# disanda/Deep-GAN-Encoders

Measured on AMD Instinct MI355X. Metric: encoder-train images/sec (E_align_s2 step, StyleGAN2 FFHQ-1024), higher is better.
Workload: dtype bf16; 1 GPU; E_align_s2 two-phase step, StyleGAN2-1024 G (train mode) + BE(startf=16, L=9) + LPIPS-VGG16 (seeded stand-in weights), batch 8/GPU; global_batch=8, img_size=1024, parallelism=dp1

## Files before the change

deep-gan-encoders_amd/csrc/enc_bwd_kernels.hip:

```cpp
#include <stdlib.h>
#include "common.h"
#include "../../include/dge_hip.h"

template <int NTAP>
__device__ __forceinline__ void wgrad_flush(const f32x16_t (&acc)[NTAP], float* smem, float* __restrict__ dW, int o0, int i0,
                                            int Co, int Ci, int tid, int lane, int wave) {
    float* red = smem;
    float* stage = smem + 4096;
#pragma unroll
    for (int t = 0; t < NTAP; t++) {
        __syncthreads();
#pragma unroll
        for (int r = 0; r < 16; r++) red[wave * 1024 + r * 64 + lane] = acc[t][r];
        __syncthreads();
#pragma unroll
        for (int q = 0; q < 4; q++) {
            const int e = tid + q * 256;
            const int r = e >> 6, ln = e & 63;
            const int ol = (r & 3) + 8 * (r >> 2) + 4 * (ln >> 5), il = ln & 31;
            stage[(ol * 32 + il) * NTAP + t] = (red[e] + red[1024 + e]) + (red[2048 + e] + red[3072 + e]);
        }
    }
    __syncthreads();
    const int ni = (Ci - i0 < 32 ? Ci - i0 : 32) * NTAP;
    if (det_on()) {
        const int L = 1024 * NTAP, nslots = gridDim.y;
        float* slot = det_slot(blockIdx.x, gridDim.x, blockIdx.y, nslots, L);
        for (int idx = tid; idx < L; idx += 256) slot[idx] = stage[idx];
        if (det_arrive_wg(blockIdx.x, nslots)) {
            for (int idx = tid; idx < L; idx += 256) {
                const int ol = idx / (32 * NTAP), j = idx - ol * (32 * NTAP);
                if (o0 + ol < Co && j < ni) dW[((size_t)(o0 + ol) * Ci + i0) * NTAP + j] += det_sum(blockIdx.x, nslots, L, idx);
            }
        }
        return;
    }
    for (int idx = tid; idx < 1024 * NTAP; idx += 256) {
        const int ol = idx / (32 * NTAP), j = idx - ol * (32 * NTAP);
        if (o0 + ol < Co && j < ni) atomicAdd(dW + ((size_t)(o0 + ol) * Ci + i0) * NTAP + j, stage[idx]);
    }
}

template <typename T, int KS>
__global__ __launch_bounds__(256) void conv_wgrad_kernel(const T* __restrict__ g, const T* __restrict__ X,
                                                          const float* __restrict__ sc, const float* __restrict__ sh,
                                                          float* __restrict__ dW, int B, int H, int W, int Co, int Ci,
                                                          int tiles_x, int tiles_y, int ntile_groups) {
    constexpr int TH = 8, TW = 16, HALO = KS / 2, HH = TH + 2 * HALO, HW = TW + 2 * HALO;
    constexpr int EP = Elem<T>::PER16;
    constexpr int ES = (int)sizeof(T);
    constexpr int NTAP = KS * KS;
    constexpr int GPIT = TH * TW + 16 / ES;
    constexpr int XROW = 24 * 2 / ES >= 24 ? 24 : 24;
    constexpr int XPIT = HH * XROW + 16 / ES;
    constexpr int LG_BYTES = 32 * GPIT * ES, LX_BYTES = 32 * XPIT * ES;
    constexpr int FL_BYTES = (4096 + 1024 * NTAP) * 4;
    constexpr int SM_BYTES = (LG_BYTES + LX_BYTES) > FL_BYTES ? (LG_BYTES + LX_BYTES) : FL_BYTES;
    __shared__ __attribute__((aligned(16))) unsigned char smem[SM_BYTES];
    T* lg = (T*)smem;
    T* lx = (T*)(smem + LG_BYTES);
    const int tid = threadIdx.x, lane = tid & 63, wave = tid >> 6;
    const int n_it = (Ci + 31) / 32;
    const int o0 = (blockIdx.x / n_it) * 32, i0 = (blockIdx.x % n_it) * 32;
    f32x16_t acc[NTAP];
#pragma unroll
    for (int t = 0; t < NTAP; t++)
#pragma unroll
        for (int r = 0; r < 16; r++) acc[t][r] = 0.f;
    const int ntiles = tiles_x * tiles_y * B;
    constexpr int CPR = 32 / EP;
    constexpr int NG = (TH * TW * CPR + 255) / 256, NX = (HH * HW * CPR + 255) / 256;
    __shared__ float laff[64];
    const int m = lane & 31, kg = lane >> 5;
    uint4 greg[NG], xreg[NX];
    auto load_tile = [&](int tile) {
        const int tx_i = tile % tiles_x, ty_i = (tile / tiles_x) % tiles_y, b = tile / (tiles_x * tiles_y);
        const int x0 = tx_i * TW, y0 = ty_i * TH;
#pragma unroll
        for (int k = 0; k < NG; k++) {
            const int idx = tid + k * 256;
            const int pix = idx % (TH * TW), c = idx / (TH * TW), gy = y0 + pix / TW, gx = x0 + pix % TW;
            uint4 v = make_uint4(0, 0, 0, 0);
            if (idx < TH * TW * CPR && gy < H && gx < W && o0 + c * EP < Co)
                v = *(const uint4*)(g + ((size_t)(b * H + gy) * W + gx) * Co + o0 + c * EP);
            greg[k] = v;
        }
#pragma unroll
        for (int k = 0; k < NX; k++) {
            const int idx = tid + k * 256;
            const int pix = idx % (HH * HW), c = idx / (HH * HW), hy = pix / HW, hx = pix % HW;
            const int gy = y0 + hy - HALO, gx = x0 + hx - HALO;
            uint4 v = make_uint4(0, 0, 0, 0);
            if (idx < HH * HW * CPR && gy >= 0 && gy < H && gx >= 0 && gx < W && i0 + c * EP < Ci)
                v = *(const uint4*)(X + ((size_t)(b * H + gy) * W + gx) * Ci + i0 + c * EP);
            xreg[k] = v;
        }
    };
    int b_aff = -1;
    if ((int)blockIdx.y < ntiles) load_tile(blockIdx.y);
    for (int tile = blockIdx.y; tile < ntiles; tile += ntile_groups) {
        const int tx_i = tile % tiles_x, ty_i = (tile / tiles_x) % tiles_y, b = tile / (tiles_x * tiles_y);
        const int x0 = tx_i * TW, y0 = ty_i * TH;
        __syncthreads();
        if (sc && b != b_aff) {
            if (tid < 64) {
                const int ch = i0 + (tid & 31);
                laff[tid] = ch < Ci ? (tid < 32 ? sc[b * Ci + ch] : sh[b * Ci + ch]) : 0.f;
            }
            b_aff = b;
            __syncthreads();
        }
#pragma unroll
        for (int k = 0; k < NG; k++) {
            const int idx = tid + k * 256;
            if (idx < TH * TW * CPR) {
                const int pix = idx % (TH * TW), c = idx / (TH * TW);
                const T* e = (const T*)&greg[k];
#pragma unroll
                for (int q = 0; q < EP; q++) lg[(c * EP + q) * GPIT + pix] = e[q];
            }
        }
#pragma unroll
        for (int k = 0; k < NX; k++) {
            const int idx = tid + k * 256;
            if (idx < HH * HW * CPR) {
                const int pix = idx % (HH * HW), c = idx / (HH * HW), hy = pix / HW, hx = pix % HW;
                const int gy = y0 + hy - HALO, gx = x0 + hx - HALO;
                uint4 v = xreg[k];
                if (sc && gy >= 0 && gy < H && gx >= 0 && gx < W) {
                    float f[EP];
                    unpack16(v, f, (T*)nullptr);
#pragma unroll
                    for (int q = 0; q < EP; q++) f[q] = f[q] * laff[c * EP + q] + laff[32 + c * EP + q];
                    v = pack16(f, (T*)nullptr);
                }
                const T* e = (const T*)&v;
#pragma unroll
                for (int q = 0; q < EP; q++) lx[(c * EP + q) * XPIT + hy * XROW + hx] = e[q];
            }
        }
        __syncthreads();
        if (tile + ntile_groups < ntiles) load_tile(tile + ntile_groups);
        constexpr int RW = TH / 4;
#pragma unroll
        for (int rr = 0; rr < RW; rr++) {
            const int row = RW * wave + rr;
            if constexpr (sizeof(T) == 2) {
                const uint4 a = *(const uint4*)(lg + m * GPIT + row * TW + kg * 8);
#pragma unroll
                for (int dy = 0; dy < KS; dy++) {
                    const T* xr = lx + m * XPIT + (row + dy) * XROW + kg * 8;
                    const uint4 v0 = *(const uint4*)xr;
                    if constexpr (KS == 3) {
                        const uint32_t v1 = *(const uint32_t*)(xr + 8);
                        const uint4 b1 = make_uint4(__builtin_amdgcn_alignbit(v0.y, v0.x, 16), __builtin_amdgcn_alignbit(v0.z, v0.y, 16),
                                                    __builtin_amdgcn_alignbit(v0.w, v0.z, 16), __builtin_amdgcn_alignbit(v1, v0.w, 16));
                        const uint4 b2 = make_uint4(v0.y, v0.z, v0.w, v1);
                        acc[dy * 3 + 0] = __builtin_amdgcn_mfma_f32_32x32x16_bf16(*(const bf16x8_t*)&a, *(const bf16x8_t*)&v0, acc[dy * 3 + 0], 0, 0, 0);
                        acc[dy * 3 + 1] = __builtin_amdgcn_mfma_f32_32x32x16_bf16(*(const bf16x8_t*)&a, *(const bf16x8_t*)&b1, acc[dy * 3 + 1], 0, 0, 0);
                        acc[dy * 3 + 2] = __builtin_amdgcn_mfma_f32_32x32x16_bf16(*(const bf16x8_t*)&a, *(const bf16x8_t*)&b2, acc[dy * 3 + 2], 0, 0, 0);
                    } else {
                        acc[0] = __builtin_amdgcn_mfma_f32_32x32x16_bf16(*(const bf16x8_t*)&a, *(const bf16x8_t*)&v0, acc[0], 0, 0, 0);
                    }
                }
            } else {
                const float* ar = (const float*)lg + m * GPIT + row * TW + kg * 8;
                float af[8];
                *(uint4*)&af[0] = *(const uint4*)ar; *(uint4*)&af[4] = *(const uint4*)(ar + 4);
#pragma unroll
                for (int dy = 0; dy < KS; dy++) {
                    const float* xr = (const float*)lx + m * XPIT + (row + dy) * XROW + kg * 8;
                    float xf[12];
                    *(uint4*)&xf[0] = *(const uint4*)xr; *(uint4*)&xf[4] = *(const uint4*)(xr + 4);
                    if constexpr (KS == 3) *(uint4*)&xf[8] = *(const uint4*)(xr + 8);
#pragma unroll
                    for (int dx = 0; dx < KS; dx++)
#pragma unroll
                        for (int j = 0; j < 8; j++)
                            acc[dy * KS + dx] = __builtin_amdgcn_mfma_f32_32x32x2f32(af[j], xf[j + dx], acc[dy * KS + dx], 0, 0, 0);
                }
            }
        }
    }
    wgrad_flush<NTAP>(acc, (float*)smem, dW, o0, i0, Co, Ci, tid, lane, wave);
}

typedef short v4s_t __attribute__((ext_vector_type(4)));
template <int KS, int TH>
__global__ __launch_bounds__(256) void conv_wgrad_tr_kernel(const bf16_t* __restrict__ g, const bf16_t* __restrict__ X,
                                                             const float* __restrict__ sc, const float* __restrict__ sh,
                                                             float* __restrict__ dW, int B, int H, int W, int Co, int Ci,
                                                             int tiles_x, int tiles_y, int ntile_groups) {
    constexpr int TW = 16, HALO = KS / 2, HH = TH + 2 * HALO, HW = TW + 2 * HALO;
    constexpr int NTAP = KS * KS;
    constexpr int LG_BYTES = TH * TW * 64, LX_BYTES = (HH * HW + 4) * 64;
    constexpr int FL_BYTES = (4096 + 1024 * NTAP) * 4;
    constexpr int SM_BYTES = (LG_BYTES + LX_BYTES) > FL_BYTES ? (LG_BYTES + LX_BYTES) : FL_BYTES;
    __shared__ __attribute__((aligned(256))) unsigned char smem[SM_BYTES];
    __shared__ float laff[64];
    unsigned char* lg = smem;
    unsigned char* lx = smem + LG_BYTES;
    const int tid = threadIdx.x, lane = tid & 63;
    const int wave = __builtin_amdgcn_readfirstlane(tid >> 6);
    const int n_it = (Ci + 31) / 32;
    const int o0 = (blockIdx.x / n_it) * 32, i0 = (blockIdx.x % n_it) * 32;
    f32x16_t acc[NTAP];
#pragma unroll
    for (int t = 0; t < NTAP; t++)
#pragma unroll
        for (int r = 0; r < 16; r++) acc[t][r] = 0.f;
    const int ntiles = tiles_x * tiles_y * B;
    constexpr int NG = TH * TW * 4 / 256, NX = (HH * HW * 4 + 255) / 256;
    const int cch = tid & 3;
    const bool gc_ok = o0 + cch * 8 < Co, xc_ok = i0 + cch * 8 < Ci;
    uint4 greg[NG], xreg[NX];
    unsigned xin = 0;
    auto load_tile = [&](int tile) {
        const int tx_i = tile % tiles_x, ty_i = (tile / tiles_x) % tiles_y, b = tile / (tiles_x * tiles_y);
        const int x0 = tx_i * TW, y0 = ty_i * TH;
        const bf16_t* gb = g + (size_t)b * H * W * Co + o0 + cch * 8;
        const bf16_t* xb = X + (size_t)b * H * W * Ci + i0 + cch * 8;
#pragma unroll
        for (int k = 0; k < NG; k++) {
            const int pix = (tid >> 2) + k * 64, gy = y0 + pix / TW, gx = x0 + pix % TW;
            uint4 v = make_uint4(0, 0, 0, 0);
            if ((gy < H) & (gx < W) & gc_ok) v = *(const uint4*)(gb + (gy * W + gx) * Co);
            greg[k] = v;
        }
        xin = 0;
#pragma unroll
        for (int k = 0; k < NX; k++) {
            const int pix = (tid >> 2) + k * 64, hy = pix / HW, hx = pix % HW;
            const int gy = y0 + hy - HALO, gx = x0 + hx - HALO;
            const bool in = (pix < HH * HW) & ((unsigned)gy < (unsigned)H) & ((unsigned)gx < (unsigned)W) & xc_ok;
            uint4 v = make_uint4(0, 0, 0, 0);
            if (in) v = *(const uint4*)(xb + (gy * W + gx) * Ci);
            xin |= (in ? 1u : 0u) << k;
            xreg[k] = v;
        }
    };
    const int grp = lane >> 4, li = lane & 15;
    const int frag_off = ((grp >> 1) * 8 + (li >> 2)) * 64 + (grp & 1) * 32 + (li & 3) * 8;
    typedef __attribute__((address_space(3))) v4s_t* lds_v4s_ptr;
    auto trd = [&](const unsigned char* base, int byte_off) {
        return __builtin_amdgcn_ds_read_tr16_b64_v4i16((lds_v4s_ptr)(base + byte_off));
    };
    int b_aff = -1;
    if ((int)blockIdx.y < ntiles) load_tile(blockIdx.y);
    for (int tile = blockIdx.y; tile < ntiles; tile += ntile_groups) {
        const int b = tile / (tiles_x * tiles_y);
        __syncthreads();
        if (sc && b != b_aff) {
            if (tid < 64) {
                const int ch = i0 + (tid & 31);
                laff[tid] = ch < Ci ? (tid < 32 ? sc[b * Ci + ch] : sh[b * Ci + ch]) : 0.f;
            }
            b_aff = b;
            __syncthreads();
        }
#pragma unroll
        for (int k = 0; k < NG; k++) *(uint4*)(lg + (tid + k * 256) * 16) = greg[k];
#pragma unroll
        for (int k = 0; k < NX; k++) {
            if (NX * 256 == HH * HW * 4 || tid + k * 256 < HH * HW * 4) {
                uint4 v = xreg[k];
                if (sc && ((xin >> k) & 1u)) {
                    float f[8];
                    unpack16(v, f, (bf16_t*)nullptr);
#pragma unroll
                    for (int q = 0; q < 8; q++) f[q] = f[q] * laff[cch * 8 + q] + laff[32 + cch * 8 + q];
                    v = pack16(f, (bf16_t*)nullptr);
                }
                *(uint4*)(lx + (tid + k * 256) * 16) = v;
            }
        }
        __syncthreads();
        if (tile + ntile_groups < ntiles) load_tile(tile + ntile_groups);
        constexpr int RW = TH / 4;
#pragma unroll
        for (int rr = 0; rr < RW; rr++) {
            const int row = RW * wave + rr;
            const unsigned char* ga = lg + row * TW * 64 + frag_off;
            const v4s_t a0 = trd(ga, 0), a1 = trd(ga, 4 * 64);
            const uint2 a01 = *(const uint2*)&a0, a23 = *(const uint2*)&a1;
            const uint4 av = make_uint4(a01.x, a01.y, a23.x, a23.y);
            const bf16x8_t a = *(const bf16x8_t*)&av;
#pragma unroll
            for (int dy = 0; dy < KS; dy++) {
                const unsigned char* xa = lx + (row + dy) * HW * 64 + frag_off;
                const v4s_t q0 = trd(xa, 0), q1 = trd(xa, 4 * 64);
                const uint2 w01 = *(const uint2*)&q0, w23 = *(const uint2*)&q1;
                const uint4 v0 = make_uint4(w01.x, w01.y, w23.x, w23.y);
                if constexpr (KS == 3) {
                    const v4s_t q2 = trd(xa, 8 * 64);
                    const uint32_t w4 = (*(const uint2*)&q2).x;
                    const uint4 b1 = make_uint4(__builtin_amdgcn_alignbit(v0.y, v0.x, 16), __builtin_amdgcn_alignbit(v0.z, v0.y, 16),
                                                __builtin_amdgcn_alignbit(v0.w, v0.z, 16), __builtin_amdgcn_alignbit(w4, v0.w, 16));
                    const uint4 b2 = make_uint4(v0.y, v0.z, v0.w, w4);
                    acc[dy * 3 + 0] = __builtin_amdgcn_mfma_f32_32x32x16_bf16(a, *(const bf16x8_t*)&v0, acc[dy * 3 + 0], 0, 0, 0);
                    acc[dy * 3 + 1] = __builtin_amdgcn_mfma_f32_32x32x16_bf16(a, *(const bf16x8_t*)&b1, acc[dy * 3 + 1], 0, 0, 0);
                    acc[dy * 3 + 2] = __builtin_amdgcn_mfma_f32_32x32x16_bf16(a, *(const bf16x8_t*)&b2, acc[dy * 3 + 2], 0, 0, 0);
                } else {
                    acc[0] = __builtin_amdgcn_mfma_f32_32x32x16_bf16(a, *(const bf16x8_t*)&v0, acc[0], 0, 0, 0);
                }
            }
        }
    }
    wgrad_flush<NTAP>(acc, (float*)smem, dW, o0, i0, Co, Ci, tid, lane, wave);
}

template <typename T, int NS>
__global__ __launch_bounds__(256) void act_bwd_kernel(const T* __restrict__ gup, const T* __restrict__ a,
                                                       const float* __restrict__ noise, T* __restrict__ gpre,
                                                       float* __restrict__ red_out, int H, int W, int C, int pool, float scale, float slope) {
    constexpr int EP = Elem<T>::PER16;
    __shared__ float red[256 * NS * EP];
    const int b = blockIdx.y;
    const int cpt = C / EP, ppi = 256 / cpt;
    const int chunk = threadIdx.x % cpt, slot = threadIdx.x / cpt;
    const int HW = H * W, UW = pool ? W / 2 : W, UHW = pool ? HW / 4 : HW;
    const float raw_w = pool ? 0.25f : 1.f;
    float s[NS][EP];
#pragma unroll
    for (int k = 0; k < NS; k++)
#pragma unroll
        for (int e = 0; e < EP; e++) s[k][e] = 0.f;
    for (int p0 = blockIdx.x * ppi; p0 < HW; p0 += gridDim.x * ppi) {
        const int p = p0 + slot;
        if (slot < ppi && p < HW) {
            const int q = pool ? (p / W / 2) * UW + (p % W) / 2 : p;
            float g[EP], av[EP];
            unpack16(*(const uint4*)(gup + ((size_t)b * UHW + q) * C + chunk * EP), g, (T*)nullptr);
            unpack16(*(const uint4*)(a + ((size_t)b * HW + p) * C + chunk * EP), av, (T*)nullptr);
            const float nz = noise ? noise[(size_t)b * HW + p] : 0.f;
#pragma unroll
            for (int e = 0; e < EP; e++) {
                if constexpr (NS == 3) s[2][e] += raw_w * g[e];
                g[e] = scale * g[e] * (av[e] > 0.f ? 1.f : slope);
                s[0][e] += g[e]; s[1][e] += g[e] * nz;
            }
            *(uint4*)(gpre + ((size_t)b * HW + p) * C + chunk * EP) = pack16(g, (T*)nullptr);
        }
    }
    if (red_out) block_chan_flush<EP, NS>(s, cpt, ppi, red_out + (size_t)b * C * NS, C, red);
}

template <typename T, int NS>
__global__ __launch_bounds__(256) void act_bwd_mask_kernel(const T* __restrict__ gup, const unsigned* __restrict__ mask,
                                                            const float* __restrict__ noise, T* __restrict__ gpre,
                                                            float* __restrict__ red_out, int H, int W, int C, float scale, float slope) {
    constexpr int EP = Elem<T>::PER16;
    __shared__ float red[256 * NS * EP];
    const int b = blockIdx.y;
    const int cpt = C / EP, ppi = 256 / cpt;
    const int chunk = threadIdx.x % cpt, slot = threadIdx.x / cpt;
    const int UW = W / 2, UHW = (H / 2) * UW, HW = H * W;
    float s[NS][EP];
#pragma unroll
    for (int k = 0; k < NS; k++)
#pragma unroll
        for (int e = 0; e < EP; e++) s[k][e] = 0.f;
    const int stride = gridDim.x * ppi;
    for (int q0 = blockIdx.x * ppi; q0 < UHW; q0 += 2 * stride) {
        const int qq[2] = {q0 + slot, q0 + slot + stride};
        bool ok[2]; uint4 gv[2]; unsigned mv[2]; int p00[2]; float nzv[2][4];
#pragma unroll
        for (int h = 0; h < 2; h++) {
            ok[h] = slot < ppi && qq[h] < UHW;
            gv[h] = make_uint4(0, 0, 0, 0); mv[h] = 0; p00[h] = 0;
#pragma unroll
            for (int c4 = 0; c4 < 4; c4++) nzv[h][c4] = 0.f;
            if (ok[h]) {
                gv[h] = *(const uint4*)(gup + ((size_t)b * UHW + qq[h]) * C + chunk * EP);
                mv[h] = mask[((size_t)b * UHW + qq[h]) * cpt + chunk];
                const int oy = qq[h] / UW, ox = qq[h] - oy * UW;
                p00[h] = (2 * oy) * W + 2 * ox;
                if (noise) {
#pragma unroll
                    for (int c4 = 0; c4 < 4; c4++) nzv[h][c4] = noise[(size_t)b * HW + p00[h] + (c4 >> 1) * W + (c4 & 1)];
                }
            }
        }
#pragma unroll
        for (int h = 0; h < 2; h++) {
            if (!ok[h]) continue;
            float g[EP];
            unpack16(gv[h], g, (T*)nullptr);
            const unsigned m = mv[h];
#pragma unroll
            for (int e = 0; e < EP; e++) { if constexpr (NS == 3) s[2][e] += g[e]; g[e] *= scale; }
#pragma unroll
            for (int c4 = 0; c4 < 4; c4++) {
                const int p = p00[h] + (c4 >> 1) * W + (c4 & 1);
                const float nz = nzv[h][c4];
                float o[EP];
#pragma unroll
                for (int e = 0; e < EP; e++) {
                    o[e] = g[e] * (((m >> (c4 * EP + e)) & 1u) ? 1.f : slope);
                    s[0][e] += o[e]; s[1][e] += o[e] * nz;
                }
                *(uint4*)(gpre + ((size_t)b * HW + p) * C + chunk * EP) = pack16(o, (T*)nullptr);
            }
        }
    }
    if (red_out) block_chan_flush<EP, NS>(s, cpt, ppi, red_out + (size_t)b * C * NS, C, red);
}

__global__ void in_bwd_coef_kernel(const float* __restrict__ dots, const float* __restrict__ gms, const float* __restrict__ musig,
                                   const float* __restrict__ sc, const float* __restrict__ sh, float* __restrict__ coef,
                                   int B, int C, float inv_n, int nslot) {
    const int idx = blockIdx.x * blockDim.x + threadIdx.x;
    if (idx >= B * C) return;
    const int b = idx / C, c = idx % C;
    const float r = sc[idx], s = sh[idx];
    float S2 = 0.f, S1 = 0.f;
    if (dots) {
        const float2 ss = sum_slot_pairs(dots + (size_t)idx * 2, (size_t)B * C * 2, nslot);
        S2 = ss.x; S1 = ss.y;
    }
    const float m1 = S1 * inv_n, m2 = (r * S2 + s * S1) * inv_n;
    const float mu = musig[(size_t)b * 2 * C + c], sg = musig[(size_t)b * 2 * C + C + c];
    const float gmu = gms ? gms[(size_t)b * 2 * C + c] : 0.f, gsg = gms ? gms[(size_t)b * 2 * C + C + c] : 0.f;
    const float k = sg > 0.f ? gsg * inv_n / sg : 0.f;
    coef[(size_t)idx * 3 + 0] = r;
    coef[(size_t)idx * 3 + 1] = -r * r * m2 + k;
    coef[(size_t)idx * 3 + 2] = -r * m1 - r * m2 * s + gmu * inv_n - k * mu;
}

struct InCoefSrc { const float* dots; const float* gms; const float* musig; const float* sc; const float* sh; int nslot, B; float inv_n; };
template <typename T, bool FR>
__global__ __launch_bounds__(256) void in_bwd_kernel(const T* __restrict__ gy, const T* __restrict__ X, const float* __restrict__ coef,
                                                      const T* __restrict__ extra, const float* __restrict__ noise,
                                                      T* __restrict__ gout, float* __restrict__ red_out, int H, int W, int C,
                                                      int extra_pool, float extra_scale, int act, InCoefSrc cs,
                                                      const float* __restrict__ img, float* __restrict__ fr_out) {
    constexpr int EP = Elem<T>::PER16;
    __shared__ float red[256 * (FR ? 4 : 2) * EP];
    __shared__ float lcoef[3 * 512];
    const int b = blockIdx.y;
    const int cpt = C / EP, ppi = 256 / cpt;
    const int chunk = threadIdx.x % cpt, slot = threadIdx.x / cpt;
    const int HW = H * W, UW = extra_pool ? W / 2 : W, UHW = extra_pool ? HW / 4 : HW;
    float s[FR ? 4 : 2][EP], A[EP], Bc[EP], Cc[EP];
    if (!coef) {
        for (int c = threadIdx.x; c < C; c += 256) {
            const int idx = b * C + c;
            const float r = cs.sc[idx], sft = cs.sh[idx];
            float S2 = 0.f, S1 = 0.f;
            if (cs.dots) { const float2 ss = sum_slot_pairs(cs.dots + (size_t)idx * 2, (size_t)cs.B * C * 2, cs.nslot); S2 = ss.x; S1 = ss.y; }
            const float m1 = S1 * cs.inv_n, m2 = (r * S2 + sft * S1) * cs.inv_n;
            const float mu = cs.musig[(size_t)b * 2 * C + c], sg = cs.musig[(size_t)b * 2 * C + C + c];
            const float gmu = cs.gms ? cs.gms[(size_t)b * 2 * C + c] : 0.f, gsg = cs.gms ? cs.gms[(size_t)b * 2 * C + C + c] : 0.f;
            const float k = sg > 0.f ? gsg * cs.inv_n / sg : 0.f;
            lcoef[c * 3 + 0] = r;
            lcoef[c * 3 + 1] = -r * r * m2 + k;
            lcoef[c * 3 + 2] = -r * m1 - r * m2 * sft + gmu * cs.inv_n - k * mu;
        }
        __syncthreads();
    }
#pragma unroll
    for (int e = 0; e < EP; e++) {
// ... 231 lines not shown
            unpack16(ev[h], ex, (T*)nullptr);
            a[h][0] = a[h][1] = a[h][2] = 0.f;
            if (ok[h]) {
#pragma unroll
                for (int e = 0; e < EP; e++) {
                    float ge;
                    if constexpr (AFF) ge = A[e] * g[e];
                    else ge = A[e] * g[e] + Bc[e] * xv[e] + Cc[e];
                    if (extra) ge += extra_scale * ex[e];
                    const float gp = ge * (xv[e] > 0.f ? 1.f : 0.2f);
                    a[h][0] += gp * wr[0][e]; a[h][1] += gp * wr[1][e]; a[h][2] += gp * wr[2][e];
                    if constexpr (FR) { s[0][e] += gp * im[h][0]; s[1][e] += gp * im[h][1]; s[2][e] += gp * im[h][2]; s[3][e] += gp; }
                }
            }
        }
        for (int m = 1; m < cpt && m < 64; m <<= 1) {
#pragma unroll
            for (int h = 0; h < 2; h++)
#pragma unroll
                for (int k = 0; k < 3; k++) a[h][k] += __shfl_xor(a[h][k], m, 64);
        }
        if (cpt > 64) {
            const int wave = threadIdx.x >> 6, wpp = cpt >> 6;
            if ((threadIdx.x & 63) == 0) {
#pragma unroll
                for (int h = 0; h < 2; h++)
#pragma unroll
                    for (int k = 0; k < 3; k++) xw[(h * 4 + wave) * 3 + k] = a[h][k];
            }
            __syncthreads();
            if (chunk == 0) {
#pragma unroll
                for (int h = 0; h < 2; h++)
#pragma unroll
                    for (int k = 0; k < 3; k++) {
                        float t = 0.f;
                        for (int j = 0; j < wpp; j++) t += xw[(h * 4 + wave + j) * 3 + k];
                        a[h][k] = t;
                    }
            }
            __syncthreads();
        }
        if (chunk == 0) {
#pragma unroll
            for (int h = 0; h < 2; h++) {
                if (!ok[h]) continue;
#pragma unroll
                for (int k = 0; k < 3; k++) gimg[((size_t)b * 3 + k) * HW + pp[h]] = a[h][k];
            }
        }
    }
    if constexpr (FR) block_chan_flush<EP, 4>(s, cpt, ppi, fr_out + (size_t)b * C * 4, C, red);
}

template <typename T>
__global__ __launch_bounds__(256) void nearest_up2_kernel(const T* __restrict__ x, T* __restrict__ y, int H, int W, int C, float scale, long total16) {
    constexpr int EP = Elem<T>::PER16;
    const int cpt = C / EP;
    for (long idx = blockIdx.x * 256L + threadIdx.x; idx < total16; idx += (long)gridDim.x * 256) {
        const int chunk = idx % cpt;
        const long pix = idx / cpt;
        const int ox = pix % (2 * W), oy = (pix / (2 * W)) % (2 * H);
        const long b = pix / ((long)4 * H * W);
        float v[EP];
        unpack16(*(const uint4*)(x + ((b * H + (oy >> 1)) * W + (ox >> 1)) * C + chunk * EP), v, (T*)nullptr);
#pragma unroll
        for (int e = 0; e < EP; e++) v[e] *= scale;
        *(uint4*)(y + pix * C + chunk * EP) = pack16(v, (T*)nullptr);
    }
}

__global__ void dense_wgrad_kernel(const float* __restrict__ gy, int ldgy, const float* __restrict__ x, int ldx,
                                   float* __restrict__ gW, float* __restrict__ gb, int B, int O, int I, int accumulate) {
    const long idx = blockIdx.x * 256L + threadIdx.x;
    if (idx >= (long)O * I) return;
    const int o = idx / I, i = idx % I;
    float s = 0.f, sb = 0.f;
    for (int b = 0; b < B; b++) { const float g = gy[(size_t)b * ldgy + o]; s += g * x[(size_t)b * ldx + i]; sb += g; }
    gW[idx] = accumulate ? gW[idx] + s : s;
    if (gb && i == 0) gb[o] = accumulate ? gb[o] + sb : sb;
}

struct HeadEntry { const float* W; long moff, woff; int I, gcol, boff, pad; const float* bias; };
__global__ __launch_bounds__(1024) void head_bwd_data_kernel(const HeadEntry* __restrict__ tab, const float* __restrict__ g, int ldg,
                                                             float* __restrict__ gms_all, int O) {
    __shared__ float part[16][64];
    const HeadEntry e = tab[blockIdx.z];
    const int lane = threadIdx.x & 63, wave = threadIdx.x >> 6;
    const int k = blockIdx.x * 64 + lane, b = blockIdx.y;
    if (blockIdx.x * 64 >= e.I) return;
    const int per = (O + 15) / 16, o0 = wave * per, o1 = min(O, o0 + per);
    float acc[8];
#pragma unroll
    for (int j = 0; j < 8; j++) acc[j] = 0.f;
    if (k < e.I) {
        const float* gr = g + (size_t)b * ldg + e.gcol;
        int o = o0;
        for (; o + 7 < o1; o += 8) {
#pragma unroll
            for (int j = 0; j < 8; j++) acc[j] += gr[o + j] * e.W[(size_t)(o + j) * e.I + k];
        }
        for (; o < o1; o++) acc[0] += gr[o] * e.W[(size_t)o * e.I + k];
    }
    part[wave][lane] = ((acc[0] + acc[1]) + (acc[2] + acc[3])) + ((acc[4] + acc[5]) + (acc[6] + acc[7]));
    __syncthreads();
    if (wave == 0 && k < e.I) {
        float s = 0.f;
#pragma unroll
        for (int j = 0; j < 16; j++) s += part[j][lane];
        gms_all[e.moff + (size_t)b * e.I + k] = s;
    }
}
__global__ void head_bwd_param_kernel(const HeadEntry* __restrict__ tab, const float* __restrict__ g, int ldg,
                                      const float* __restrict__ musig_all, float* __restrict__ gw_all, float* __restrict__ gb_all,
                                      int B, int O) {
    const HeadEntry e = tab[blockIdx.y];
    const int total = O * e.I;
    for (int idx = blockIdx.x * 256 + threadIdx.x; idx < total; idx += gridDim.x * 256) {
        const int o = idx / e.I, i = idx - o * e.I;
        float s = 0.f, sb = 0.f;
        for (int b = 0; b < B; b++) {
            const float gv = g[(size_t)b * ldg + e.gcol + o];
            s += gv * musig_all[e.moff + (size_t)b * e.I + i]; sb += gv;
        }
        gw_all[e.woff + idx] = s;
        if (i == 0) gb_all[e.boff + o] = sb;
    }
}

#define CHAN_OK(C, ep) ((C) % (ep) == 0 && (C) / (ep) <= 256 && 256 % ((C) / (ep)) == 0)

int dge_wgrad_dma_try(const void* g, const void* x, const float* sc, const float* sh, float* dw, int B, int H, int W, int cout, int cin,
                      const float* wdot, float* dots, int dots_slots, hipStream_t s);
extern "C" int dge_conv_wgrad_dots(const void* g, const void* x, const float* in_scale, const float* in_shift, float* dw, const float* w,
                                   float* dots, int dots_slots, int B, int H, int W, int cout, int cin, int dtype, hipStream_t s) {
    DGE_CHECK(g && x && dw && w && dots && in_scale && in_shift && dots_slots >= 1, "conv_wgrad_dots: null tensor");
    if (dtype != DGE_BF16) return 1;
    return dge_wgrad_dma_try(g, x, in_scale, in_shift, dw, B, H, W, cout, cin, w, dots, dots_slots, s);
}
extern "C" int dge_conv_wgrad(const void* g, const void* x, const float* in_scale, const float* in_shift, float* dw, int B, int H,
                              int W, int cout, int cin, int ksize, int dtype, hipStream_t s) {
    DGE_CHECK(ksize == 1 || ksize == 3, "conv_wgrad: ksize %d unsupported", ksize);
    const int ep = dtype == DGE_BF16 ? 8 : 4;
    DGE_CHECK(cout % ep == 0 && cin % ep == 0, "conv_wgrad: channels must be multiples of %d", ep);
    DGE_CHECK((in_scale == nullptr) == (in_shift == nullptr), "conv_wgrad: in_scale and in_shift go together");
    if (dtype == DGE_BF16 && ksize == 3) {
        const int r = dge_wgrad_dma_try(g, x, in_scale, in_shift, dw, B, H, W, cout, cin, nullptr, nullptr, 1, s);
        if (r <= 0) return r;
    }
    const bool tall = dtype == DGE_BF16 && H >= 16 && !dge_env().wgrad_th8;
    const int tx = (W + 15) / 16, ty = tall ? (H + 15) / 16 : (H + 7) / 8;
    const int ntiles = tx * ty * B;
    const int noi = ((cout + 31) / 32) * ((cin + 31) / 32);
    int groups = 512 / noi; if (groups < 1) groups = 1;
    if (dge_env().wgrad_groups > 0) groups = dge_env().wgrad_groups;
    if (groups > ntiles) groups = ntiles;
    dim3 grid(noi, groups);
    if (dtype == DGE_BF16) dge_note_kernel("conv_wgrad_tr<%d,%d>", ksize, tall ? 16 : 8);
    else dge_note_kernel("conv_wgrad<f32,%d>", ksize);
#define WG(T, KS) hipLaunchKernelGGL((conv_wgrad_kernel<T, KS>), grid, dim3(256), 0, s, (const T*)g, (const T*)x, in_scale, in_shift, dw, B, H, W, cout, cin, tx, ty, groups)
    if (dtype == DGE_BF16) {
#define WT(KS, TH) hipLaunchKernelGGL((conv_wgrad_tr_kernel<KS, TH>), grid, dim3(256), 0, s, (const bf16_t*)g, (const bf16_t*)x, in_scale, in_shift, dw, B, H, W, cout, cin, tx, ty, groups)
        if (ksize == 3) { if (tall) WT(3, 16); else WT(3, 8); }
        else { if (tall) WT(1, 16); else WT(1, 8); }
#undef WT
    }
    else { if (ksize == 3) WG(float, 3); else WG(float, 1); }
#undef WG
    DGE_LAUNCH_CHECK("conv_wgrad");
    return 0;
}

__global__ __launch_bounds__(256) void head_fwd_kernel(const HeadEntry* __restrict__ tab, const float* __restrict__ musig_all,
                                                       float* __restrict__ w, int ldw, int B, int O) {
    const HeadEntry e = tab[blockIdx.y];
    const int wave = (blockIdx.x * 256 + threadIdx.x) >> 6, lane = threadIdx.x & 63;
    if (wave >= B * O) return;
    const int b = wave / O, o = wave - b * O;
    const float* xr = musig_all + e.moff + (size_t)b * e.I;
    const float* wr = e.W + (size_t)o * e.I;
    float s = 0.f;
    for (int i = lane; i < e.I; i += 64) s = fmaf(xr[i], wr[i], s);
    s = wave_sum(s);
    if (lane == 0) w[(size_t)b * ldw + e.gcol + o] = s + (e.bias ? e.bias[o] : 0.f);
}
extern "C" int dge_heads_fwd(const void* dev_entries, int n, const float* musig_all, float* w, int ldw, int B, int O, hipStream_t s) {
    DGE_CHECK(n >= 1 && n <= 65535 && B >= 1 && O >= 1, "heads_fwd: bad sizes");
    hipLaunchKernelGGL(head_fwd_kernel, dim3((B * O * 64 + 255) / 256, n), dim3(256), 0, s, (const HeadEntry*)dev_entries, musig_all, w, ldw, B, O);
    DGE_LAUNCH_CHECK("heads_fwd");
    return 0;
}

extern "C" int dge_head_entry_size(void) { return (int)sizeof(HeadEntry); }
extern "C" int dge_heads_bwd(const void* dev_entries, int n, int max_I, const float* g, int ldg, const float* musig_all, float* gms_all,
                             float* gw_all, float* gb_all, int B, int O, hipStream_t s) {
    DGE_CHECK(n >= 1 && n <= 65535 && B >= 1 && B <= 65535 && O >= 1 && max_I >= 1, "heads_bwd: bad sizes");
    hipLaunchKernelGGL(head_bwd_data_kernel, dim3((max_I + 63) / 64, B, n), dim3(1024), 0, s, (const HeadEntry*)dev_entries, g, ldg, gms_all, O);
    hipLaunchKernelGGL(head_bwd_param_kernel, dim3(64, n), dim3(256), 0, s, (const HeadEntry*)dev_entries, g, ldg, musig_all, gw_all,
                       gb_all, B, O);
    DGE_LAUNCH_CHECK("heads_bwd");
    return 0;
}

struct HeadRowsEntry { const float* W; const float* bias; long moff, woff; int I, row_a, row_b, boff; };
constexpr int HEAD_ROWS_MAX_O = 1024;

__global__ __launch_bounds__(256) void head_rows_fwd_kernel(const HeadRowsEntry* __restrict__ tab, const float* __restrict__ musig_all,
                                                            float* __restrict__ w, long ldb, long ldr, int nrows, int B, int O) {
    const HeadRowsEntry e = tab[blockIdx.y];
    const int wave = (blockIdx.x * 256 + threadIdx.x) >> 6, lane = threadIdx.x & 63;
    if (wave >= B * O) return;
    const int b = wave / O, o = wave % O;
    const float* xr = musig_all + e.moff + (size_t)b * e.I;
    const float* wr = e.W + (size_t)o * e.I;
    float s = 0.f;
    for (int i = lane; i < e.I; i += 64) { const float xv = xr[i]; s += xv * wr[i]; }
    s = wave_sum(s);
    if (lane == 0) {
        const float v = s + (e.bias ? e.bias[o] : 0.f);
        if ((unsigned)e.row_a < (unsigned)nrows) w[(size_t)b * ldb + (size_t)e.row_a * ldr + o] = v;
        if ((unsigned)e.row_b < (unsigned)nrows) w[(size_t)b * ldb + (size_t)e.row_b * ldr + o] = v;
    }
}

__global__ __launch_bounds__(1024) void head_rows_bwd_data_kernel(const HeadRowsEntry* __restrict__ tab, const float* __restrict__ g,
                                                                  long ldb, long ldr, int nrows, float* __restrict__ gms_all, int O) {
    __shared__ float gs[HEAD_ROWS_MAX_O];
    __shared__ float part[16][64];
    const HeadRowsEntry e = tab[blockIdx.z];
    const int lane = threadIdx.x & 63, wave = threadIdx.x >> 6;
    const int k = blockIdx.x * 64 + lane, b = blockIdx.y;
    if (blockIdx.x * 64 >= e.I) return;
    const bool ha = (unsigned)e.row_a < (unsigned)nrows, hb = (unsigned)e.row_b < (unsigned)nrows;
    for (int o = threadIdx.x; o < O; o += 1024) {
        float v = ha ? g[(size_t)b * ldb + (size_t)e.row_a * ldr + o] : 0.f;
        if (hb) v += g[(size_t)b * ldb + (size_t)e.row_b * ldr + o];
        gs[o] = v;
    }
    __syncthreads();
    const int per = (O + 15) / 16, o0 = min(O, wave * per), o1 = min(O, o0 + per);
    float acc[8];
#pragma unroll
    for (int j = 0; j < 8; j++) acc[j] = 0.f;
    if (k < e.I) {
        int o = o0;
        for (; o + 7 < o1; o += 8) {
#pragma unroll
            for (int j = 0; j < 8; j++) acc[j] += gs[o + j] * e.W[(size_t)(o + j) * e.I + k];
        }
        for (; o < o1; o++) acc[0] += gs[o] * e.W[(size_t)o * e.I + k];
    }
    part[wave][lane] = ((acc[0] + acc[1]) + (acc[2] + acc[3])) + ((acc[4] + acc[5]) + (acc[6] + acc[7]));
    __syncthreads();
    if (wave == 0 && k < e.I) {
        float s = 0.f;
#pragma unroll
        for (int j = 0; j < 16; j++) s += part[j][lane];
        gms_all[e.moff + (size_t)b * e.I + k] = s;
    }
}
__global__ __launch_bounds__(256) void head_rows_bwd_param_kernel(const HeadRowsEntry* __restrict__ tab, const float* __restrict__ g,
                                                                  long ldb, long ldr, int nrows, const float* __restrict__ musig_all,
                                                                  float* __restrict__ gw_all, float* __restrict__ gb_all, int B, int O) {
    const HeadRowsEntry e = tab[blockIdx.y];
    const bool ha = (unsigned)e.row_a < (unsigned)nrows, hb = (unsigned)e.row_b < (unsigned)nrows;
    const int total = O * e.I;
    for (int idx = blockIdx.x * 256 + threadIdx.x; idx < total; idx += gridDim.x * 256) {
        const int o = idx / e.I, i = idx - o * e.I;
        float s = 0.f, sb = 0.f;
        for (int b = 0; b < B; b++) {
            float gv = ha ? g[(size_t)b * ldb + (size_t)e.row_a * ldr + o] : 0.f;
            if (hb) gv += g[(size_t)b * ldb + (size_t)e.row_b * ldr + o];
            s += gv * musig_all[e.moff + (size_t)b * e.I + i]; sb += gv;
        }
        gw_all[e.woff + idx] = s;
        if (i == 0) gb_all[e.boff + o] = sb;
    }
}

extern "C" int dge_head_rows_entry_size(void) { return (int)sizeof(HeadRowsEntry); }
extern "C" int dge_heads_rows_fwd(const void* dev_entries, int n, const float* musig_all, float* w, long ldb, long ldr, int nrows,
                                  int B, int O, hipStream_t s) {
    DGE_CHECK(dev_entries && musig_all && w, "heads_rows_fwd: null tensor");
    DGE_CHECK(n >= 1 && n <= 65535 && B >= 1 && O >= 1 && nrows >= 1 && (long)B * O <= (1L << 24), "heads_rows_fwd: bad sizes");
    DGE_CHECK(ldr >= O && ldb >= O, "heads_rows_fwd: w strides (%ld, %ld) are below the row length %d", ldb, ldr, O);
    hipLaunchKernelGGL(head_rows_fwd_kernel, dim3((unsigned)(((long)B * O * 64 + 255) / 256), n), dim3(256), 0, s,
                       (const HeadRowsEntry*)dev_entries, musig_all, w, ldb, ldr, nrows, B, O);
    DGE_LAUNCH_CHECK("heads_rows_fwd");
    return 0;
}
extern "C" int dge_heads_rows_bwd(const void* dev_entries, int n, int max_I, const float* g, long ldb, long ldr, int nrows,
                                  const float* musig_all, float* gms_all, float* gw_all, float* gb_all, int B, int O, hipStream_t s) {
    DGE_CHECK(dev_entries && g && gms_all, "heads_rows_bwd: null tensor");
    DGE_CHECK(n >= 1 && n <= 65535 && B >= 1 && B <= 65535 && O >= 1 && O <= HEAD_ROWS_MAX_O && max_I >= 1 && nrows >= 1,
              "heads_rows_bwd: bad sizes (O <= %d)", HEAD_ROWS_MAX_O);
    DGE_CHECK((gw_all == nullptr) == (gb_all == nullptr) && (gw_all == nullptr || musig_all != nullptr),
              "heads_rows_bwd: gw_all, gb_all and musig_all go together (all null: the data gradient alone)");
    hipLaunchKernelGGL(head_rows_bwd_data_kernel, dim3((max_I + 63) / 64, B, n), dim3(1024), 0, s, (const HeadRowsEntry*)dev_entries, g,
                       ldb, ldr, nrows, gms_all, O);
    if (gw_all)
        hipLaunchKernelGGL(head_rows_bwd_param_kernel, dim3(64, n), dim3(256), 0, s, (const HeadRowsEntry*)dev_entries, g, ldb, ldr, nrows,
                           musig_all, gw_all, gb_all, B, O);
    DGE_LAUNCH_CHECK("heads_rows_bwd");
    return 0;
}

extern "C" int dge_act_bwd(const void* gup, const void* a, const float* noise, void* gpre, float* red, int red_cols, int B, int H,
                           int W, int C, int pool, float scale, float slope, int dtype, hipStream_t s) {
    const int ep = dtype == DGE_BF16 ? 8 : 4;
    DGE_CHECK(CHAN_OK(C, ep), "act_bwd: unsupported channel count %d", C);
    DGE_CHECK(red_cols == 2 || red_cols == 3, "act_bwd: red_cols must be 2 or 3 (got %d)", red_cols);
    dim3 grid(dge_stream_grid(H * W, 256 / (C / ep), B), B);
#define AB(T, NS) hipLaunchKernelGGL((act_bwd_kernel<T, NS>), grid, dim3(256), 0, s, (const T*)gup, (const T*)a, noise, (T*)gpre, red, H, W, C, pool, scale, slope)
    if (dtype == DGE_BF16) { if (red_cols == 3) AB(bf16_t, 3); else AB(bf16_t, 2); }
    else { if (red_cols == 3) AB(float, 3); else AB(float, 2); }
#undef AB
    DGE_LAUNCH_CHECK("act_bwd");
// ... 154 lines not shown
```

Measured before the change: 387.4 images/sec.

## Run two wave-teams per block in bf16 3x3 wgrad, add placement and non-atomic flush

For bf16 3x3 weight-gradient convolution the kernel now launches 512-thread blocks holding two independent 4-wave teams. Each team walks an interleaved subset of tiles with its own LDS buffers, and the two teams' accumulators are reduced together in the flush. This halves the number of block partials that have to be combined for each weight tile. For 1x1 kernels an optional swizzled block placement groups tile-groups of the same output tile on nearby blocks. When there is only one tile group, the flush does a plain read-add-write instead of atomics. In exchange, LDS use per block and register pressure go up, and the teams need matched barrier counts, which adds dummy-sync bookkeeping.

New measurement: 389.7 images/sec (median of 6 runs). Within noise of the previous version (+0.6%).

```diff
diff --git a/deep-gan-encoders_amd/csrc/enc_bwd_kernels.hip b/deep-gan-encoders_amd/csrc/enc_bwd_kernels.hip
--- a/deep-gan-encoders_amd/csrc/enc_bwd_kernels.hip
+++ b/deep-gan-encoders_amd/csrc/enc_bwd_kernels.hip
@@ -2,11 +2,13 @@
 #include "common.h"
 #include "../../include/dge_hip.h"
 
-template <int NTAP>
+template <int NTAP, int NW = 4>
 __device__ __forceinline__ void wgrad_flush(const f32x16_t (&acc)[NTAP], float* smem, float* __restrict__ dW, int o0, int i0,
-                                            int Co, int Ci, int tid, int lane, int wave) {
+                                            int Co, int Ci, int tid, int lane, int wave, int dom, int ndom, int slot, int nslots,
+                                            bool single) {
+    constexpr int NT = NW * 64;
     float* red = smem;
-    float* stage = smem + 4096;
+    float* stage = smem + NW * 1024;
 #pragma unroll
     for (int t = 0; t < NTAP; t++) {
         __syncthreads();
@@ -14,28 +16,45 @@
         for (int r = 0; r < 16; r++) red[wave * 1024 + r * 64 + lane] = acc[t][r];
         __syncthreads();
 #pragma unroll
-        for (int q = 0; q < 4; q++) {
-            const int e = tid + q * 256;
+        for (int q = 0; q < 1024 / NT; q++) {
+            const int e = tid + q * NT;
             const int r = e >> 6, ln = e & 63;
             const int ol = (r & 3) + 8 * (r >> 2) + 4 * (ln >> 5), il = ln & 31;
-            stage[(ol * 32 + il) * NTAP + t] = (red[e] + red[1024 + e]) + (red[2048 + e] + red[3072 + e]);
+            float sum = (red[e] + red[1024 + e]) + (red[2048 + e] + red[3072 + e]);
+            if constexpr (NW == 8) sum += (red[4096 + e] + red[5120 + e]) + (red[6144 + e] + red[7168 + e]);
+            stage[(ol * 32 + il) * NTAP + t] = sum;
         }
     }
     __syncthreads();
     const int ni = (Ci - i0 < 32 ? Ci - i0 : 32) * NTAP;
     if (det_on()) {
-        const int L = 1024 * NTAP, nslots = gridDim.y;
-        float* slot = det_slot(blockIdx.x, gridDim.x, blockIdx.y, nslots, L);
-        for (int idx = tid; idx < L; idx += 256) slot[idx] = stage[idx];
-        if (det_arrive_wg(blockIdx.x, nslots)) {
-            for (int idx = tid; idx < L; idx += 256) {
+        const int L = 1024 * NTAP;
+        float* slotp = det_slot(dom, ndom, slot, nslots, L);
+        for (int idx = tid; idx < L; idx += NT) slotp[idx] = stage[idx];
+        if (det_arrive_wg(dom, nslots)) {
+            for (int idx = tid; idx < L; idx += NT) {
                 const int ol = idx / (32 * NTAP), j = idx - ol * (32 * NTAP);
-                if (o0 + ol < Co && j < ni) dW[((size_t)(o0 + ol) * Ci + i0) * NTAP + j] += det_sum(blockIdx.x, nslots, L, idx);
+                if (o0 + ol < Co && j < ni) dW[((size_t)(o0 + ol) * Ci + i0) * NTAP + j] += det_sum(dom, nslots, L, idx);
             }
         }
         return;
     }
-    for (int idx = tid; idx < 1024 * NTAP; idx += 256) {
+    if (single) {
+        constexpr int NI = 1024 * NTAP / NT;
+        float old[NI];
+#pragma unroll
+        for (int k = 0; k < NI; k++) {
+            const int idx = tid + k * NT, ol = idx / (32 * NTAP), j = idx - ol * (32 * NTAP);
+            old[k] = (o0 + ol < Co && j < ni) ? dW[((size_t)(o0 + ol) * Ci + i0) * NTAP + j] : 0.f;
+        }
+#pragma unroll
+        for (int k = 0; k < NI; k++) {
+            const int idx = tid + k * NT, ol = idx / (32 * NTAP), j = idx - ol * (32 * NTAP);
+            if (o0 + ol < Co && j < ni) dW[((size_t)(o0 + ol) * Ci + i0) * NTAP + j] = old[k] + stage[idx];
+        }
+        return;
+    }
+    for (int idx = tid; idx < 1024 * NTAP; idx += NT) {
         const int ol = idx / (32 * NTAP), j = idx - ol * (32 * NTAP);
         if (o0 + ol < Co && j < ni) atomicAdd(dW + ((size_t)(o0 + ol) * Ci + i0) * NTAP + j, stage[idx]);
     }
@@ -182,28 +201,36 @@
             }
         }
     }
-    wgrad_flush<NTAP>(acc, (float*)smem, dW, o0, i0, Co, Ci, tid, lane, wave);
+    wgrad_flush<NTAP>(acc, (float*)smem, dW, o0, i0, Co, Ci, tid, lane, wave, blockIdx.x, gridDim.x, blockIdx.y, gridDim.y, false);
 }
 
 typedef short v4s_t __attribute__((ext_vector_type(4)));
-template <int KS, int TH>
-__global__ __launch_bounds__(256) void conv_wgrad_tr_kernel(const bf16_t* __restrict__ g, const bf16_t* __restrict__ X,
-                                                             const float* __restrict__ sc, const float* __restrict__ sh,
-                                                             float* __restrict__ dW, int B, int H, int W, int Co, int Ci,
-                                                             int tiles_x, int tiles_y, int ntile_groups) {
+template <int KS, int TH, int NH>
+__global__ __launch_bounds__(256 * NH) void conv_wgrad_tr_kernel(const bf16_t* __restrict__ g, const bf16_t* __restrict__ X,
+                                                                  const float* __restrict__ sc, const float* __restrict__ sh,
+                                                                  float* __restrict__ dW, int B, int H, int W, int Co, int Ci,
+                                                                  int tiles_x, int tiles_y, int ntile_groups, int noi, int place) {
     constexpr int TW = 16, HALO = KS / 2, HH = TH + 2 * HALO, HW = TW + 2 * HALO;
     constexpr int NTAP = KS * KS;
     constexpr int LG_BYTES = TH * TW * 64, LX_BYTES = (HH * HW + 4) * 64;
-    constexpr int FL_BYTES = (4096 + 1024 * NTAP) * 4;
-    constexpr int SM_BYTES = (LG_BYTES + LX_BYTES) > FL_BYTES ? (LG_BYTES + LX_BYTES) : FL_BYTES;
+    constexpr int FL_BYTES = (NH * 4096 + 1024 * NTAP) * 4;
+    constexpr int SM_BYTES = NH * (LG_BYTES + LX_BYTES) > FL_BYTES ? NH * (LG_BYTES + LX_BYTES) : FL_BYTES;
     __shared__ __attribute__((aligned(256))) unsigned char smem[SM_BYTES];
-    __shared__ float laff[64];
-    unsigned char* lg = smem;
-    unsigned char* lx = smem + LG_BYTES;
+    __shared__ float laff_all[NH * 64];
+    int oi = blockIdx.x, grp = blockIdx.y;
+    if (place) {
+        const int v = blockIdx.x >> 3;
+        oi = v % noi; grp = (v / noi) * 8 + (blockIdx.x & 7);
+        if (grp >= ntile_groups) return;
+    }
     const int tid = threadIdx.x, lane = tid & 63;
     const int wave = __builtin_amdgcn_readfirstlane(tid >> 6);
+    const int team = NH == 1 ? 0 : wave >> 2, wv = wave & 3, ttid = tid & 255;
+    unsigned char* lg = smem + team * (LG_BYTES + LX_BYTES);
+    unsigned char* lx = lg + LG_BYTES;
+    float* laff = laff_all + team * 64;
     const int n_it = (Ci + 31) / 32;
-    const int o0 = (blockIdx.x / n_it) * 32, i0 = (blockIdx.x % n_it) * 32;
+    const int o0 = (oi / n_it) * 32, i0 = (oi % n_it) * 32;
     f32x16_t acc[NTAP];
 #pragma unroll
     for (int t = 0; t < NTAP; t++)
@@ -211,7 +238,7 @@
         for (int r = 0; r < 16; r++) acc[t][r] = 0.f;
     const int ntiles = tiles_x * tiles_y * B;
     constexpr int NG = TH * TW * 4 / 256, NX = (HH * HW * 4 + 255) / 256;
-    const int cch = tid & 3;
+    const int cch = ttid & 3;
     const bool gc_ok = o0 + cch * 8 < Co, xc_ok = i0 + cch * 8 < Ci;
     uint4 greg[NG], xreg[NX];
     unsigned xin = 0;
@@ -222,7 +249,7 @@
         const bf16_t* xb = X + (size_t)b * H * W * Ci + i0 + cch * 8;
 #pragma unroll
         for (int k = 0; k < NG; k++) {
-            const int pix = (tid >> 2) + k * 64, gy = y0 + pix / TW, gx = x0 + pix % TW;
+            const int pix = (ttid >> 2) + k * 64, gy = y0 + pix / TW, gx = x0 + pix % TW;
             uint4 v = make_uint4(0, 0, 0, 0);
             if ((gy < H) & (gx < W) & gc_ok) v = *(const uint4*)(gb + (gy * W + gx) * Co);
             greg[k] = v;
@@ -230,7 +257,7 @@
         xin = 0;
 #pragma unroll
         for (int k = 0; k < NX; k++) {
-            const int pix = (tid >> 2) + k * 64, hy = pix / HW, hx = pix % HW;
+            const int pix = (ttid >> 2) + k * 64, hy = pix / HW, hx = pix % HW;
             const int gy = y0 + hy - HALO, gx = x0 + hx - HALO;
             const bool in = (pix < HH * HW) & ((unsigned)gy < (unsigned)H) & ((unsigned)gx < (unsigned)W) & xc_ok;
             uint4 v = make_uint4(0, 0, 0, 0);
@@ -239,74 +266,91 @@
             xreg[k] = v;
         }
     };
-    const int grp = lane >> 4, li = lane & 15;
-    const int frag_off = ((grp >> 1) * 8 + (li >> 2)) * 64 + (grp & 1) * 32 + (li & 3) * 8;
+    const int fg = lane >> 4, li = lane & 15;
+    const int frag_off = ((fg >> 1) * 8 + (li >> 2)) * 64 + (fg & 1) * 32 + (li & 3) * 8;
     typedef __attribute__((address_space(3))) v4s_t* lds_v4s_ptr;
     auto trd = [&](const unsigned char* base, int byte_off) {
         return __builtin_amdgcn_ds_read_tr16_b64_v4i16((lds_v4s_ptr)(base + byte_off));
     };
-    int b_aff = -1;
-    if ((int)blockIdx.y < ntiles) load_tile(blockIdx.y);
-    for (int tile = blockIdx.y; tile < ntiles; tile += ntile_groups) {
-        const int b = tile / (tiles_x * tiles_y);
+    const int first = grp + team * ntile_groups, stride = NH * ntile_groups;
+    const int n_mine = first < ntiles ? (ntiles - first + stride - 1) / stride : 0;
+    const int iters = (ntiles - grp + stride - 1) / stride;
+    auto load_aff = [&](int b) {
+        if (ttid < 64) {
+            const int ch = i0 + (ttid & 31);
+            laff[ttid] = ch < Ci ? (ttid < 32 ? sc[b * Ci + ch] : sh[b * Ci + ch]) : 0.f;
+        }
+    };
+    const int tps = tiles_x * tiles_y;
+    if (n_mine > 0) {
+        load_tile(first);
+        if (sc) load_aff(first / tps);
+    }
+    __syncthreads();
+    if (NH == 2 && team == 1) __syncthreads();
+    for (int j = 0; j < n_mine; j++) {
+        const int tile = first + j * stride;
+        {
+            {
+#pragma unroll
+                for (int k = 0; k < NG; k++) *(uint4*)(lg + (ttid + k * 256) * 16) = greg[k];
+#pragma unroll
+                for (int k = 0; k < NX; k++) {
+                    if (NX * 256 == HH * HW * 4 || ttid + k * 256 < HH * HW * 4) {
+                        uint4 v = xreg[k];
+                        if (sc && ((xin >> k) & 1u)) {
+                            float f[8];
+                            unpack16(v, f, (bf16_t*)nullptr);
+#pragma unroll
+                            for (int e = 0; e < 8; e++) f[e] = f[e] * laff[cch * 8 + e] + laff[32 + cch * 8 + e];
+                            v = pack16(f, (bf16_t*)nullptr);
+                        }
+                        *(uint4*)(lx + (ttid + k * 256) * 16) = v;
+                    }
+                }
+            }
+            __syncthreads();
+            {
+                if (j + 1 < n_mine) {
+                    load_tile(tile + stride);
+                    if (sc && (tile + stride) / tps != tile / tps) load_aff((tile + stride) / tps);
+                }
+                constexpr int RW = TH / 4;
+#pragma unroll
+                for (int rr = 0; rr < RW; rr++) {
+                    const int row = RW * wv + rr;
+                    const unsigned char* ga = lg + row * TW * 64 + frag_off;
+                    const v4s_t a0 = trd(ga, 0), a1 = trd(ga, 4 * 64);
+                    const uint2 a01 = *(const uint2*)&a0, a23 = *(const uint2*)&a1;
+                    const uint4 av = make_uint4(a01.x, a01.y, a23.x, a23.y);
+                    const bf16x8_t a = *(const bf16x8_t*)&av;
+#pragma unroll
+                    for (int dy = 0; dy < KS; dy++) {
+                        const unsigned char* xa = lx + (row + dy) * HW * 64 + frag_off;
+                        const v4s_t q0 = trd(xa, 0), q1 = trd(xa, 4 * 64);
+                        const uint2 w01 = *(const uint2*)&q0, w23 = *(const uint2*)&q1;
+                        const uint4 v0 = make_uint4(w01.x, w01.y, w23.x, w23.y);
+                        if constexpr (KS == 3) {
+                            const v4s_t q2 = trd(xa, 8 * 64);
+                            const uint32_t w4 = (*(const uint2*)&q2).x;
+                            const uint4 b1 = make_uint4(__builtin_amdgcn_alignbit(v0.y, v0.x, 16), __builtin_amdgcn_alignbit(v0.z, v0.y, 16),
+                                                        __builtin_amdgcn_alignbit(v0.w, v0.z, 16), __builtin_amdgcn_alignbit(w4, v0.w, 16));
+                            const uint4 b2 = make_uint4(v0.y, v0.z, v0.w, w4);
+                            acc[dy * 3 + 0] = __builtin_amdgcn_mfma_f32_32x32x16_bf16(a, *(const bf16x8_t*)&v0, acc[dy * 3 + 0], 0, 0, 0);
+                            acc[dy * 3 + 1] = __builtin_amdgcn_mfma_f32_32x32x16_bf16(a, *(const bf16x8_t*)&b1, acc[dy * 3 + 1], 0, 0, 0);
+                            acc[dy * 3 + 2] = __builtin_amdgcn_mfma_f32_32x32x16_bf16(a, *(const bf16x8_t*)&b2, acc[dy * 3 + 2], 0, 0, 0);
+                        } else {
+                            acc[0] = __builtin_amdgcn_mfma_f32_32x32x16_bf16(a, *(const bf16x8_t*)&v0, acc[0], 0, 0, 0);
+                        }
+                    }
+                }
+            }
+        }
         __syncthreads();
-        if (sc && b != b_aff) {
-            if (tid < 64) {
-                const int ch = i0 + (tid & 31);
-                laff[tid] = ch < Ci ? (tid < 32 ? sc[b * Ci + ch] : sh[b * Ci + ch]) : 0.f;
-            }
-            b_aff = b;
-            __syncthreads();
-        }
-#pragma unroll
-        for (int k = 0; k < NG; k++) *(uint4*)(lg + (tid + k * 256) * 16) = greg[k];
-#pragma unroll
-        for (int k = 0; k < NX; k++) {
-            if (NX * 256 == HH * HW * 4 || tid + k * 256 < HH * HW * 4) {
-                uint4 v = xreg[k];
-                if (sc && ((xin >> k) & 1u)) {
-                    float f[8];
-                    unpack16(v, f, (bf16_t*)nullptr);
-#pragma unroll
-                    for (int q = 0; q < 8; q++) f[q] = f[q] * laff[cch * 8 + q] + laff[32 + cch * 8 + q];
-                    v = pack16(f, (bf16_t*)nullptr);
-                }
-                *(uint4*)(lx + (tid + k * 256) * 16) = v;
-            }
-        }
-        __syncthreads();
-        if (tile + ntile_groups < ntiles) load_tile(tile + ntile_groups);
-        constexpr int RW = TH / 4;
-#pragma unroll
-        for (int rr = 0; rr < RW; rr++) {
-            const int row = RW * wave + rr;
-            const unsigned char* ga = lg + row * TW * 64 + frag_off;
-            const v4s_t a0 = trd(ga, 0), a1 = trd(ga, 4 * 64);
-            const uint2 a01 = *(const uint2*)&a0, a23 = *(const uint2*)&a1;
-            const uint4 av = make_uint4(a01.x, a01.y, a23.x, a23.y);
-            const bf16x8_t a = *(const bf16x8_t*)&av;
-#pragma unroll
-            for (int dy = 0; dy < KS; dy++) {
-                const unsigned char* xa = lx + (row + dy) * HW * 64 + frag_off;
-                const v4s_t q0 = trd(xa, 0), q1 = trd(xa, 4 * 64);
-                const uint2 w01 = *(const uint2*)&q0, w23 = *(const uint2*)&q1;
-                const uint4 v0 = make_uint4(w01.x, w01.y, w23.x, w23.y);
-                if constexpr (KS == 3) {
-                    const v4s_t q2 = trd(xa, 8 * 64);
-                    const uint32_t w4 = (*(const uint2*)&q2).x;
-                    const uint4 b1 = make_uint4(__builtin_amdgcn_alignbit(v0.y, v0.x, 16), __builtin_amdgcn_alignbit(v0.z, v0.y, 16),
-                                                __builtin_amdgcn_alignbit(v0.w, v0.z, 16), __builtin_amdgcn_alignbit(w4, v0.w, 16));
-                    const uint4 b2 = make_uint4(v0.y, v0.z, v0.w, w4);
-                    acc[dy * 3 + 0] = __builtin_amdgcn_mfma_f32_32x32x16_bf16(a, *(const bf16x8_t*)&v0, acc[dy * 3 + 0], 0, 0, 0);
-                    acc[dy * 3 + 1] = __builtin_amdgcn_mfma_f32_32x32x16_bf16(a, *(const bf16x8_t*)&b1, acc[dy * 3 + 1], 0, 0, 0);
-                    acc[dy * 3 + 2] = __builtin_amdgcn_mfma_f32_32x32x16_bf16(a, *(const bf16x8_t*)&b2, acc[dy * 3 + 2], 0, 0, 0);
-                } else {
-                    acc[0] = __builtin_amdgcn_mfma_f32_32x32x16_bf16(a, *(const bf16x8_t*)&v0, acc[0], 0, 0, 0);
-                }
-            }
-        }
-    }
-    wgrad_flush<NTAP>(acc, (float*)smem, dW, o0, i0, Co, Ci, tid, lane, wave);
+    }
+    for (int j = n_mine; j < iters; j++) { __syncthreads(); __syncthreads(); }
+    if (NH == 2 && team == 0) __syncthreads();
+    wgrad_flush<NTAP, 4 * NH>(acc, (float*)smem, dW, o0, i0, Co, Ci, tid, lane, wave, oi, noi, grp, ntile_groups, ntile_groups == 1);
 }
 
 template <typename T, int NS>
@@ -844,17 +888,21 @@
     const int tx = (W + 15) / 16, ty = tall ? (H + 15) / 16 : (H + 7) / 8;
     const int ntiles = tx * ty * B;
     const int noi = ((cout + 31) / 32) * ((cin + 31) / 32);
-    int groups = 512 / noi; if (groups < 1) groups = 1;
+    const int nh = dtype == DGE_BF16 && ksize == 3 ? 2 : 1;
+    int groups = 512 / nh / noi; if (groups < 1) groups = 1;
+    const bool place = dtype == DGE_BF16 && ksize == 1 && dge_det_fits(1LL << 40, 1, 1);
+    if (place) groups = (groups + 7) / 8 * 8;
     if (dge_env().wgrad_groups > 0) groups = dge_env().wgrad_groups;
-    if (groups > ntiles) groups = ntiles;
+    if (groups > (ntiles + nh - 1) / nh) groups = (ntiles + nh - 1) / nh;
     dim3 grid(noi, groups);
+    if (place) grid = dim3(noi * ((groups + 7) / 8 * 8), 1);
     if (dtype == DGE_BF16) dge_note_kernel("conv_wgrad_tr<%d,%d>", ksize, tall ? 16 : 8);
     else dge_note_kernel("conv_wgrad<f32,%d>", ksize);
 #define WG(T, KS) hipLaunchKernelGGL((conv_wgrad_kernel<T, KS>), grid, dim3(256), 0, s, (const T*)g, (const T*)x, in_scale, in_shift, dw, B, H, W, cout, cin, tx, ty, groups)
     if (dtype == DGE_BF16) {
-#define WT(KS, TH) hipLaunchKernelGGL((conv_wgrad_tr_kernel<KS, TH>), grid, dim3(256), 0, s, (const bf16_t*)g, (const bf16_t*)x, in_scale, in_shift, dw, B, H, W, cout, cin, tx, ty, groups)
-        if (ksize == 3) { if (tall) WT(3, 16); else WT(3, 8); }
-        else { if (tall) WT(1, 16); else WT(1, 8); }
+#define WT(KS, TH, NH) hipLaunchKernelGGL((conv_wgrad_tr_kernel<KS, TH, NH>), grid, dim3(256 * NH), 0, s, (const bf16_t*)g, (const bf16_t*)x, in_scale, in_shift, dw, B, H, W, cout, cin, tx, ty, groups, noi, place ? 1 : 0)
+        if (ksize == 3) { if (tall) WT(3, 16, 2); else WT(3, 8, 2); }
+        else { if (tall) WT(1, 16, 1); else WT(1, 8, 1); }
 #undef WT
     }
     else { if (ksize == 3) WG(float, 3); else WG(float, 1); }
```
